# NyanCAD/CedarSim.jl

Measured on AMD Instinct MI355X. Metric: newton_iters_per_sec, higher is better.
Workload: dtype f64

## Files before the change

cedarsim.jl_amd/csrc/ch_engine.hip:

```cpp
#include <hip/hip_runtime.h>
#include <hip/hip_ext.h>

#include <algorithm>
#include <atomic>
#include <chrono>
#include <cmath>
#include <cstdio>
#include <cstring>
#include <map>
#include <memory>
#include <new>
#include <stdexcept>
#include <string>
#include <array>
#include <vector>

#include "../../include/cedarhip.h"
#include "ch_analysis.hpp"
#include "ch_bsim4.hpp"
#include "ch_dc_start.hpp"
#include "ch_device_mem.hpp"
#include "ch_env.hpp"
#include "ch_gather_plan.hpp"
#include "ch_kernels.hpp"
// ... 22 lines not shown
  const double* dev_values = nullptr; int64_t dev_n = 0;
  ch_stats stats;
  int status = CH_OK;
  int n_obs = 0, S = 1;
  std::vector<double> sens; int n_par = 0;
};

struct PersistConsts; struct PersistIo; struct PersistLaunch; struct PersistRun; struct PersistStep;
struct RowStore;
struct TranSens;
struct ch_circuit;

struct Structure {
  DevBuf<int> d_comp_class, d_comp_uofs, d_comp_dofs, d_gl_ptr, d_dkind, d_dterm, d_dsrc, d_dhdev, d_obs_unk, d_unk_obs;
  DevBuf<unsigned long long> d_stamps; DevBuf<ClassMeta> d_classes; DevBuf<unsigned char> d_dmask;
  DevBuf<int> d_dvac, d_va_mod, d_va_pofs, d_va_cofs;
  int n_va_inst = 0; size_t vac_total = 0; std::vector<ClassMeta> h_cms;
  std::vector<int> obs_primary;
  std::vector<int> needed_src;
  std::vector<int> dev_src;
  int n_dev_src() const { return std::max<int>(1, (int)dev_src.size()); }
  int block_threads = 64, lu_variant = 16;
  bool wide_split = false; int wide_l = 0, wide_other = 0;
  size_t lds_doubles_fixed = 0, lds_extra_bytes = 0, lds_plan_bytes = 0;
 private: friend struct ch_circuit;
  void class_blobs(const Description& D, std::vector<int>& blob) {
    h_cms.clear();
    int max_slots = 0;
    for (size_t ci = 0; ci < D.A.classes.size(); ++ci) {
      const CompClass& c = D.A.classes[ci];
      ClassMeta m; std::memset(&m, 0, sizeof(m));
      m.nc = c.nc; m.ndev = c.ndev; m.nonlinear = c.nonlinear ? 1 : 0;
      m.n_mat_src = (int)c.mat_src.size(); m.n_vec_src = (int)c.vec_src.size();
      while (blob.size() & 3) blob.push_back(0);
      m.blob_ofs = (int)blob.size();
      blob.insert(blob.end(), c.mat_ptr.begin(), c.mat_ptr.end());
      blob.insert(blob.end(), c.vec_ptr.begin(), c.vec_ptr.end());
      int rep = -1;
      for (int k = 0; k < D.A.n_comp; ++k) if (D.A.comp_class[k] == (int)ci) { rep = k; break; }
      int ns = 0;
      {
        std::vector<int> lanes;
        bool big = false;
        for (int d = 0; d < c.ndev; ++d) {
          const EDev& e = D.A.edev[D.A.comp_dofs[rep] + d];
          if (e.kind != K_VA) continue;
          if (va_gen::MODULES[D.dev[e.hdev].ipar[0]].n_params >= 64) big = true;
// ... 15 lines not shown
      std::vector<uint16_t> h16(c.mat_src); h16.insert(h16.end(), c.vec_src.begin(), c.vec_src.end());
      if (h16.size() & 1) h16.push_back(0);
      for (size_t i = 0; i < h16.size(); i += 2) blob.push_back((int)((uint32_t)h16[i] | ((uint32_t)h16[i + 1] << 16)));
      if (((int)blob.size() - m.blob_ofs) & 1) blob.push_back(0);
      m.wl_ofs = (int)blob.size() - m.blob_ofs;
      if (c.nc <= 64 && !c.vec_ptr.empty()) {
        std::vector<std::array<int, 3>> items;
        for (int i = 0; i < c.nc; ++i) {
          const int start = c.vec_ptr[i], cnt = c.vec_ptr[i + 1] - start;
          items.push_back({cnt, m.n_mat_src + start, (int)(0x8000u | (uint32_t)i)});
        }
        for (int e = 0; e < c.nc * c.nc; ++e) {
          const int start = c.mat_ptr[e], cnt = c.mat_ptr[e + 1] - start;
          if (cnt == 0 && e / c.nc != e % c.nc) continue;
          items.push_back({cnt, start, e});
        }
        std::stable_sort(items.begin(), items.end(), [](const std::array<int, 3>& x, const std::array<int, 3>& y) { return x[0] > y[0]; });
        for (const auto& it : items) { blob.push_back(it[1]); blob.push_back((int)(((uint32_t)it[0] << 16) | (uint32_t)it[2])); ++m.n_work; }
      }
      while ((blob.size() - m.blob_ofs) & 3) blob.push_back(0);
      m.blob_ints = (int)blob.size() - m.blob_ofs;
      if (m.n_work > 0) {
        GatherPlan gp;
        if (gp.build(c.nc, c.mat_ptr, c.vec_ptr, h16, m.n_mat_src)) {
          m.spare0 = (int)gp.words.size(); m.spare1 = gp.T;
          blob.insert(blob.end(), gp.words.begin(), gp.words.end());
        }
      }
      if (env_on(Env::DEBUG_BLOB)) std::fprintf(stderr, "[blob] class %zu: nc %d ndev %d slots %d mat_src %d vec_src %d work %d blob_ints %d trips %d\n", ci, m.nc, m.ndev, m.nslots, m.n_mat_src, m.n_vec_src, m.n_work, m.blob_ints, m.spare1);
      max_slots = std::max(max_slots, m.nslots);
      h_cms.push_back(m);
    }
    block_threads = std::min(256, std::max(64, ((max_slots + 63) / 64) * 64));
    lu_variant = D.A.max_nc <= 8 ? 8 : (D.A.max_nc <= 12 ? 12 : (D.A.max_nc <= 16 ? 16 : (D.A.max_nc <= 32 ? 32 : 0)));
    if (D.A.wide) lu_variant = D.A.max_nc <= 16 ? 16 : 0;
  }
  void source_lists(const Description& D, std::vector<int>& dkind, std::vector<int>& dterm, std::vector<int>& dhdev, std::vector<int>& dsrc) {
    dsrc.clear();
    dev_src.clear();
    { std::vector<int> slot_of(D.src.size(), -1);
      for (const EDev& e : D.A.edev) {
        dkind.push_back(e.kind); for (int k = 0; k < NTERM; ++k) dterm.push_back(e.term[k]); dhdev.push_back(e.hdev);
        int si = e.kind == K_VA ? D.dev[e.hdev].ipar[1] : 0;
        if (e.src >= 0) { if (slot_of[e.src] < 0) { slot_of[e.src] = (int)dev_src.size(); dev_src.push_back(e.src); } si = slot_of[e.src]; }
        dsrc.push_back(si);
      }
      std::vector<char> need(D.src.size(), 0);
// ... 11 lines not shown
      const int mod = D.dev[e.hdev].ipar[0];
      dvac[i] = (int)vac_total; vmod.push_back(mod); vpofs.push_back(D.dev[e.hdev].ipar[1]); vcofs.push_back((int)vac_total);
      vac_total += (size_t)va_gen::N_CACHE[mod];
    }
    n_va_inst = (int)vmod.size();
    if (vmod.empty()) { vmod.push_back(0); vpofs.push_back(0); vcofs.push_back(0); }
  }
  void masks_and_observables(const Description& D, std::vector<unsigned char>& dm, std::vector<int>& obs_unk, std::vector<int>& unk_obs) {
    dm.assign(D.A.n_unk, 0);
    for (int u = 0; u < D.A.n_unk; ++u) dm[u] = (D.A.diff_mask[u] ? 1 : 0) | (D.A.unk_mna[u] >= D.n_nodes ? 2 : 0) | (D.A.replica[u] ? 4 : 0);
    obs_unk.clear(); unk_obs.assign(D.A.n_unk, -1);
    obs_primary.clear();
    for (size_t o = 0; o < D.obs_kind.size(); ++o) {
      int u = -1;
      if (D.obs_kind[o] == 0) u = D.A.node_unknown[D.obs_index[o]];
      else { int b = D.dev[D.obs_index[o]].branch; u = b >= 0 ? D.A.branch_unknown[b] : -1; }
      obs_unk.push_back(u);
      int prim = (int)o;
      if (u >= 0) { if (unk_obs[u] < 0) unk_obs[u] = (int)o; else prim = unk_obs[u]; }
      obs_primary.push_back(prim);
    }
  }
  void size_lds(const Description& D) {
    lds_doubles_fixed = 0; lds_extra_bytes = 0; lds_plan_bytes = 0;
    for (size_t ci = 0; ci < D.A.classes.size(); ++ci) {
      const CompClass& c = D.A.classes[ci];
      lds_doubles_fixed = std::max(lds_doubles_fixed, (size_t)c.ndev * D.A.stride() + (size_t)c.nc * (c.nc + 1) + (size_t)c.nc * c.nc + 12 * (size_t)c.nc);
      lds_extra_bytes = std::max(lds_extra_bytes, ((size_t)h_cms[ci].blob_ints + 64) * 4 + 16);
      lds_plan_bytes = std::max(lds_plan_bytes, (size_t)h_cms[ci].spare0 * 4);
    }
  }
};
struct SampleTables : ParamTables {
  int S = 1; bool dirty = true;
  std::vector<std::vector<double>> slot_val;
  long vac_stride_ = 0;
  DevBuf<double> d_dpar, d_dmult, d_gmin, d_temp, d_mosp, d_vapar, d_vacache;
  DevBuf<int> d_dcls, d_moscls_inst, d_mc_ofs, d_mc_n, d_mc_list, d_dcls_local;
  DevBuf<BlockMeta> d_bmeta;
};
struct SourceTables { const std::vector<double>* dc; const std::vector<double>* par; };
struct NewtonState {
  DevBuf<double> d_X, d_Q, d_rate, d_kv;
  DevBuf<unsigned char> d_perm, d_active;
  DevBuf<BlockOut> d_out; PinnedBuf<BlockOut> h_out;
  PinnedBuf<Summary> h_sum; PinnedBuf<double> h_stage;
  DevEvent ev0, ev1; bool host_reduce = true; size_t lds_bytes = 0;
  int path = 1;
  NewtonArgs base;
  mutable std::vector<double> all_src; std::vector<double> sv_buf, kv_buf;
};
struct SpGrids { int gn, gd, ga, nbr; bool many; };
// ... 742 lines not shown
```

cedarsim.jl_amd/csrc/ch_engine_persist.hpp:

```cpp
#pragma once

constexpr size_t P_MAX_ENTRIES = 64, P_MAX_PWL = 2048;
inline bool ch_circuit::persist_eligible(std::string& why, bool own_steps) {
  auto no = [&](const char* m) { why = m; return false; };
  if (nwt.path != 1) return no("the circuit takes the sparse path");
  if (desc.A.n_comp < 1) return no("the circuit has no unknowns");
  if (!(stru.lu_variant == 8 || stru.lu_variant == 12 || stru.lu_variant == 16)) return no("a Jacobian block has more than 16 unknowns");
  if (desc.A.wide) {
    if (desc.A.classes.size() != 1) return no("compiled Verilog-A devices in blocks of several classes");
    if (desc.A.nb > 0) return no("compiled Verilog-A devices in a bordered form");
    if (stru.wide_split ? (stru.wide_l + stru.wide_other > 32) : (stru.h_cms[0].nslots > 64)) return no("a block's compiled devices need more evaluation lanes than a wave pair offers");
    if (own_steps && tab.S == 1 && desc.A.n_comp > 1) return no("per-block steps of one circuit with compiled Verilog-A devices");
  } else if (stru.block_threads != 64) return no("a block needs more than one wavefront of device slots");
  if (tab.max_mc > 8) return no("more than 8 MOSFET classes in a block");
  if (tab.Ssrc != 1) return no("per-sample source parameters");
  const bool wg_consts = own_steps && tab.S == 1 && desc.A.n_comp > 1;
  if (!wg_consts && (stru.needed_src.size() > (size_t)P_MAXSRC || desc.A.known.size() + (size_t)stru.n_dev_src() > P_MAX_ENTRIES)) return no("more than 64 sources / known-node and source values per attempt");
  if (!(tab.S == 1 || desc.A.n_comp == 1)) return no("several blocks per sample in a multi-sample batch");
  if (desc.A.nb > 0 && (tab.S != 1 || desc.A.border_dev.size() > 8)) return no("bordered form: one sample and at most 8 devices on the border alone");
  for (const ClassMeta& m : stru.h_cms) if ((!desc.A.wide && m.nslots > 64) || m.nc > stru.lu_variant || m.n_work <= 0 || m.spare1 <= 0) return no("a block class does not fit the one-wave register path");
  if (ps.n_cu == 0) { hipDeviceProp_t prop; if (hipGetDeviceProperties(&prop, ctx->device) != hipSuccess) return no("hipGetDeviceProperties failed"); ps.n_cu = prop.multiProcessorCount; }
  const long nblk = (long)desc.A.n_comp * tab.S;
  const int bpw = persist_bpw(nblk);
  if (nblk > (long)bpw * ps.n_cu && !own_steps) return no("more blocks than resident wavefronts (4 per CU)");
  if (!own_steps && (nblk + bpw - 1) / bpw > 256) return no("more than 256 workgroups in a grid-wide reduction");
  size_t npwl = 0; for (int i : stru.needed_src) npwl += desc.src[i].ts.size();
  if (!wg_consts && npwl > P_MAX_PWL) return no("piecewise-linear tables above 2048 points");
  return true;
}
inline int ch_circuit::persist_bpw(long nblk) const {
  if (ps.n_cu > 0 && desc.A.wide && stru.wide_split && nblk <= 2L * ps.n_cu) return 2;
  return PW;
}
inline bool ch_circuit::persist_own_steps(const ch_tran_opts& o) const {
  return ((desc.A.n_comp == 1 && tab.S > 1) || (tab.S == 1 && desc.A.n_comp > 1 && desc.A.nb == 0 && !desc.A.wide)) && o.n_saveat > 0 && o.step_control != CH_STEPS_SHARED && !env_on(Env::LOCKSTEP);
}
inline size_t ch_circuit::persist_wave_doubles(bool wg_consts) const {
  const size_t n_ent = wg_consts ? (size_t)P_MAXSRC : desc.A.known.size() + stru.n_dev_src();
  return stru.lds_doubles_fixed + 16 * (size_t)desc.A.max_nc + 10 + 48 + P_MAXSRC + n_ent + (size_t)tab.max_mc * (B4L_STRIDE + B4D_STRIDE) + (stru.lds_extra_bytes + stru.lds_plan_bytes + 7) / 8 + 2;
}
inline bool ch_circuit::persist_blob(const std::vector<int>& kn, const std::vector<int>& ds, std::vector<int>& bi, std::vector<double>& bd, std::vector<int>& need) const {
  const int nsrc = (int)desc.src.size();
  std::vector<char> nd(std::max(1, nsrc), 0);
  for (int k : kn) for (auto& tm : desc.A.known[k].terms) nd[tm.first] = 1;
  for (int j : ds) if (j < (int)stru.dev_src.size()) nd[stru.dev_src[j]] = 1;
  need.clear();
  for (int i = 0; i < nsrc; ++i) if (nd[i]) need.push_back(i);
  std::vector<int> pos(std::max(1, nsrc), -1);
  for (size_t i = 0; i < need.size(); ++i) pos[need[i]] = (int)i;
  std::vector<double> pt, py;
  bi = {(int)need.size(), (int)(kn.size() + ds.size()), 0, (int)kn.size()};
  for (int i : need) { bi.push_back(desc.src[i].kind); bi.push_back((int)pt.size()); bi.push_back((int)desc.src[i].ts.size()); pt.insert(pt.end(), desc.src[i].ts.begin(), desc.src[i].ts.end()); py.insert(py.end(), desc.src[i].ys.begin(), desc.src[i].ys.end()); }
  bi[2] = (int)pt.size();
  std::vector<int> eptr(1, 0), eidx; std::vector<double> ecoef;
  for (int k : kn) { for (auto& tm : desc.A.known[k].terms) { eidx.push_back(pos[tm.first]); ecoef.push_back(tm.second); } eptr.push_back((int)eidx.size()); }
  for (int j : ds) { if (j < (int)stru.dev_src.size()) { eidx.push_back(pos[stru.dev_src[j]]); ecoef.push_back(1.0); } eptr.push_back((int)eidx.size()); }
  bi.insert(bi.end(), eptr.begin(), eptr.end()); bi.insert(bi.end(), eidx.begin(), eidx.end());
  bd.clear();
  for (int i : need) for (int k = 0; k < CH_SRC_NPAR; ++k) bd.push_back(tab.src_par[(size_t)i * CH_SRC_NPAR + k]);
  bd.insert(bd.end(), ecoef.begin(), ecoef.end()); bd.insert(bd.end(), pt.begin(), pt.end()); bd.insert(bd.end(), py.begin(), py.end());
  for (size_t q = 4; q < bi.size(); ++q) if (bi[q] < 0) return false;
  return need.size() <= (size_t)P_MAXSRC && kn.size() + ds.size() <= P_MAX_ENTRIES && pt.size() <= P_MAX_PWL;
// ... 226 lines not shown
  pa.indep = L.own_steps ? 1 : 0;
  ps.mode = desc.A.nb > 0 ? CH_MODE_BORDERED : (L.own_steps ? CH_MODE_OWN_STEPS : CH_MODE_LOCKSTEP);
  if (dcm) {
    if (desc.A.nb == 0 || L.wg_consts) { set_err("internal: operating point on the device stepper is for the bordered form"); return CH_ERR_INTERNAL; }
    std::vector<double> sv, kv, ent;
    eval_sources(0.0, dcm->tran_mode ? 2 : 0, sv, kv);
    ent.assign(kv.begin(), kv.begin() + nk); ent.insert(ent.end(), sv.begin(), sv.begin() + nds);
    HIPCHK(ps.d_pdcent.upload(ent, ctx->stream));
    pa.dc_mode = 1; pa.dc_maxit = std::max(1, dcm->maxiters); pa.dc_abstol = dcm->abstol; pa.dc_entries = ps.d_pdcent.p;
    pa.dv_max = (!desc.A.mos_hdev.empty() || desc.A.wide) ? dcm->dv_max : 0.0;
  }
  pa.nb = desc.A.nb; pa.n_glob = desc.A.n_glob; pa.n_bdev = (int)desc.A.border_dev.size();
  for (int q = 0; q < pa.n_bdev; ++q) {
    const Analysis::BorderDev& bd = desc.A.border_dev[q];
    pa.bd_kind[q] = bd.kind; pa.bd_ta[q] = bd.ta; pa.bd_tb[q] = bd.tb;
    const double par0 = tab.dpar[(size_t)bd.hdev * tab.Spar], mult0 = tab.dmult[(size_t)bd.hdev * tab.Spar];
    pa.bd_val[q] = bd.kind == K_R ? mult0 / par0 : mult0 * par0;
  }
  pa.pair_dbg = (int)env_long(Env::PAIR_DBG, 0);
  return CH_OK;
}
inline PersistStep ch_circuit::persist_pick_kernel(PersistLaunch& L) {
  const int mode = desc.A.wide ? (L.own_steps ? PM_OWN : PM_LOCKSTEP) : desc.A.nb > 0 ? PM_BORDER : (L.own_steps ? PM_OWN : PM_LOCKSTEP);
  L.fn = persist_kernel(desc.A.wide, mode, (desc.A.wide || desc.A.nb > 0 || stru.lu_variant > 12) ? 16 : 12, L.pair);
  if (!L.fn) { set_err("internal: no device-stepper kernel for this form"); return CH_ERR_INTERNAL; }
  if (ps.attr_fn != L.fn) {
    hipFuncAttributes fa;
    HIPCHK(hipFuncGetAttributes(&fa, L.fn));
    if (fa.sharedSizeBytes <= 160 * 1024) HIPCHK(hipFuncSetAttribute(L.fn, hipFuncAttributeMaxDynamicSharedMemorySize, (int)((160 * 1024 - (int)fa.sharedSizeBytes) & ~255)));
    ps.attr_static_lds = fa.sharedSizeBytes; ps.attr_fn = L.fn;
  }
  if (L.lds + ps.attr_static_lds > 160 * 1024) { set_err("device-resident stepper: LDS footprint"); return PersistStep::declined(); }
  return CH_OK;
}
inline PersistStep ch_circuit::persist_prepare(const TranPlan& p, const ch_dc_opts* dcm, PersistLaunch& L) {
  const ch_tran_opts& o = *p.o;
  g_arena = &arena;
  LapTimer lt(host_profile);
  L.nblk = desc.A.n_comp * tab.S; L.bpw = persist_bpw(L.nblk); L.n_wg = (L.nblk + L.bpw - 1) / L.bpw;
  L.own_steps = persist_own_steps(o);
  L.wg_consts = L.own_steps && tab.S == 1 && desc.A.n_comp > 1;
  PersistConsts pc;
  if (!persist_consts(L.wg_consts, L.n_wg, L.bpw, p, pc)) return PersistStep::declined();
  L.wave_d = persist_wave_doubles(L.wg_consts);
  L.lds = (pc.max_cd + (pc.max_ci + 1) / 2 + PW * P_NREC + P_NREC + 4 + P_SCR + PW * L.wave_d) * sizeof(double);
  L.va_arena = persist_va_arena(L.bpw, L.lds);
  L.pair = desc.A.wide ? stru.wide_split : (desc.A.classes.size() == 1 && stru.h_cms[0].nslots <= 32 && !env_on(Env::PERSIST_NOPAIR));
// ... 172 lines not shown
```

cedarsim.jl_amd/csrc/ch_gather_plan.hpp:

```cpp
#pragma once
#include <algorithm>
#include <array>
#include <cstdint>
#include <vector>

namespace chip {

constexpr int GP_HEAD_INTS = 64;
constexpr unsigned GP_N_MASK = 7u, GP_END = 8u, GP_VEC = 16u;
constexpr int GP_A_SHIFT = 6, GP_C_SHIFT = 19;
constexpr unsigned GP_OFS_MASK = 0x1fffu;

struct GatherPlan {
  struct Item { int first, cnt, code; };
  int T = 0;
  int n_items = 0, total_trips = 0, max_item_trips = 0;
  int R = 0;
  std::vector<int> words;
  std::vector<int> item_lane, item_trip;
  std::vector<Item> items;

  static int trips_of(int cnt) { return cnt <= 0 ? 1 : (cnt + 3) / 4; }
  static int lower_bound_T(int total_trips, int max_item_trips) { return std::max((total_trips + 63) / 64, max_item_trips); }

  static std::vector<Item> class_items(int nc, const std::vector<int>& mat_ptr, const std::vector<int>& vec_ptr, int n_mat_src) {
    std::vector<Item> it;
    for (int i = 0; i < nc; ++i) it.push_back({n_mat_src + vec_ptr[i], vec_ptr[i + 1] - vec_ptr[i], (int)(0x8000u | (uint32_t)i)});
    for (int e = 0; e < nc * nc; ++e) {
      const int cnt = mat_ptr[e + 1] - mat_ptr[e];
      if (cnt == 0 && e / nc != e % nc) continue;
      it.push_back({mat_ptr[e], cnt, e});
    }
    std::stable_sort(it.begin(), it.end(), [](const Item& x, const Item& y) { return x.cnt > y.cnt; });
    return it;
  }

  bool build(int nc, const std::vector<int>& mat_ptr, const std::vector<int>& vec_ptr, const std::vector<uint16_t>& src16, int n_mat_src) {
    T = 0; R = 0; n_items = 0; total_trips = 0; max_item_trips = 0; words.clear(); item_lane.clear(); item_trip.clear(); items.clear();
    if (nc < 1 || nc > 64 || (int)vec_ptr.size() != nc + 1 || (int)mat_ptr.size() != nc * nc + 1) return false;
    items = class_items(nc, mat_ptr, vec_ptr, n_mat_src);
    n_items = (int)items.size();
    for (const Item& it : items) { total_trips += trips_of(it.cnt); max_item_trips = std::max(max_item_trips, trips_of(it.cnt)); }
    std::vector<int> order(n_items);
    for (int i = 0; i < n_items; ++i) order[i] = i;
    std::stable_sort(order.begin(), order.end(), [&](int x, int y) { return trips_of(items[x].cnt) > trips_of(items[y].cnt); });
    std::array<int, 64> load;
    for (int t = lower_bound_T(total_trips, max_item_trips);; ++t) {
      load.fill(0);
      item_lane.assign(n_items, -1); item_trip.assign(n_items, 0);
      bool ok = true;
      for (int i : order) {
        const int s = trips_of(items[i].cnt);
        int l = 0;
        while (l < 64 && load[l] + s > t) ++l;
        if (l == 64) { ok = false; break; }
        item_lane[i] = l; item_trip[i] = load[l]; load[l] += s;
      }
      if (ok) { T = t; break; }
    }
    std::array<int, 64> base;
    { int next = 1; for (int l = 0; l < 64; ++l) { base[l] = load[l] > 0 ? next : 0; next += load[l]; } R = (next + 3) & ~3; }
    const int lda = nc + 1;
    words.assign((size_t)GP_HEAD_INTS + 3 * (size_t)R, 0);
    int* src = words.data() + GP_HEAD_INTS; int* ctl = src + 2 * (size_t)R;
    for (int l = 0; l < 64; ++l) words[l] = (int)((uint32_t)base[l] | ((uint32_t)load[l] << 16));
    for (int i = 0; i < n_items; ++i) {
      const Item& it = items[i];
      const int l = item_lane[i], s = trips_of(it.cnt);
      const bool vec = (it.code & 0x8000) != 0;
      const int e = it.code & 0x7fff;
      const unsigned oa = vec ? (unsigned)(e * lda + nc) : (unsigned)((e / nc) * lda + e % nc);
      const unsigned oc = vec ? (unsigned)(nc * nc + 3 * nc + e) : (unsigned)e;
      for (int q = 0; q < s; ++q) {
        const int rec = base[l] + item_trip[i] + q;
        const int left = it.cnt - 4 * q, n = left < 0 ? 0 : (left > 4 ? 4 : left);
        uint16_t o[4] = {0, 0, 0, 0};
        for (int k = 0; k < n; ++k) o[k] = src16[(size_t)it.first + 4 * q + k];
        src[2 * rec] = (int)((uint32_t)o[0] | ((uint32_t)o[1] << 16));
        src[2 * rec + 1] = (int)((uint32_t)o[2] | ((uint32_t)o[3] << 16));
        unsigned c = (unsigned)n | (vec ? GP_VEC : 0u);
        if (q == s - 1) c |= GP_END | (oa << GP_A_SHIFT) | (oc << GP_C_SHIFT);
        ctl[rec] = (int)c;
      }
    }
    if (R > 0xffff || T > 0xffff) return false;
    return true;
  }
};

}
```

cedarsim.jl_amd/csrc/ch_kernels.hpp:

```cpp
#pragma once
#include <hip/hip_runtime.h>

#include "ch_analysis.hpp"
#include "ch_bsim4.hpp"
#include "ch_param_tables.hpp"
#include "_generated/va_models.hpp"

namespace chip {


struct BlockOut {
  int status;
  int iters;
  int ndiff;
  int pad;
  double e2k, e2km1, e2kp1;
  double fnorm;
};

struct Summary {
  int n_fail, max_iters, n_singular, pad;
  long long sum_iters;
  long long sum_block_iters;
  double errk, errkm1, errkp1;
// ... 352 lines not shown
#pragma unroll
  for (int k = NC - 1; k >= 0; --k) {
    if (k < nc) {
      const double xk = bcast(rhs * ipiv, piv[k]);
      if (lane == k) out = xk;
      if (mystep >= 0 && mystep < k) rhs = fma(-r[k], xk, rhs);
    }
  }
  sol = out;
  if (myrow_out) {
    int mr = lane;
#pragma unroll
    for (int k = 0; k < NC; ++k) if (k < nc && lane == k) mr = piv[k];
    *myrow_out = mr;
  }
  return true;
}

template <int K> __device__ __forceinline__ double row_bcast(double v) {
  static_assert(K >= 0 && K < 16, "row_newbcast lane");
  const double b = __builtin_amdgcn_update_dpp(v, v, 0x150 + K, 0xF, 0xF, true);
  return b;
}
template <int NC, int J> struct RowDot {
  static __device__ __forceinline__ double run(const double (&c)[NC], double x, int nc, double q) {
    if constexpr (J < NC) {
      if (J < nc) { const double xj = row_bcast<J>(x); q = fma(c[J], xj, q); }
      return RowDot<NC, J + 1>::run(c, x, nc, q);
    } else return q;
  }
};

template <int NC, int K>
struct LuStaticStep {
  static __device__ __forceinline__ void fwd(double (&r)[NC + 1], int nc, int lane, int& lkey, double& ipiv) {
    if constexpr (K < NC) {
      if (K < nc) {
        const double ipk = frcp(row_bcast<K>(r[K]));
        double pj[NC + 1];
#pragma unroll
        for (int j = K + 1; j <= NC; ++j) pj[j] = row_bcast<K>(r[j]);
        if (lane == K) ipiv = ipk;
        if (lane > K) {
          const double l = r[K] * ipk;
          lkey = max(lkey, __double2hiint(l) & 0x7fffffff);
#pragma unroll
          for (int j = K + 1; j <= NC; ++j) r[j] = fma(-l, pj[j], r[j]);
        }
      }
      LuStaticStep<NC, K + 1>::fwd(r, nc, lane, lkey, ipiv);
    }
  }
  static __device__ __forceinline__ void bwd(const double (&r)[NC + 1], int nc, int lane, double& rhs, double ipiv) {
    if constexpr (K < NC) {
      constexpr int Q = NC - 1 - K;
      if (Q < nc && Q > 0) {
        const double xk = row_bcast<Q>(rhs * ipiv);
        if (lane < Q) rhs = fma(-r[Q], xk, rhs);
      }
      LuStaticStep<NC, K + 1>::bwd(r, nc, lane, rhs, ipiv);
    }
  }
};
template <int NC>
__device__ __forceinline__ bool lu_solve_static(double (&r)[NC + 1], int nc, int lane_in, double& sol) {
  static_assert(NC <= 16, "row_newbcast spans one 16-lane row");
  int lane = lane_in;
  asm volatile("" : "+v"(lane));
  int lkey = 0; double ipiv = 0.0;
  LuStaticStep<NC, 0>::fwd(r, nc, lane, lkey, ipiv);
  if (__ballot(lane < nc && lkey > 0x40200000)) return false;
  double rhs = r[NC];
  LuStaticStep<NC, 0>::bwd(r, nc, lane, rhs, ipiv);
  sol = rhs * ipiv;
  return true;
}
struct LuFull { double sol; int myrow; int ok; };
template <int NC>
__device__ __attribute__((noinline, cold)) LuFull lu_solve_full(const double* A, int lda, int nc, int lane, int myrow) {
  double r[NC + 1];
#pragma unroll
  for (int j = 0; j <= NC; ++j) r[j] = (lane < nc && j <= nc) ? A[lane * lda + j] : 0.0;
  LuFull o; o.sol = 0.0; o.myrow = myrow;
  o.ok = lu_solve_regs<NC>(r, nc, lane, o.sol, &o.myrow) ? 1 : 0;
  return o;
}
template <int NC>
__device__ __forceinline__ bool lu_solve_block(const double* A, int lda, int nc, int lane_in, int& myrow, double& sol) {
  if constexpr (NC <= 16) {
    int lane = lane_in;
    asm volatile("" : "+v"(lane));
    const int lim = lane < nc ? nc : 0;
    const double* row = A + (lim > 0 ? myrow : 0) * lda;
    double r[NC + 1];
#pragma unroll
    for (int j = 0; j < NC; ++j) { const double v = row[j]; r[j] = j < lim ? v : 0.0; }
    { const double v = row[nc]; r[NC] = lim > 0 ? v : 0.0; }
    if (lu_solve_static<NC>(r, nc, lane_in, sol)) return true;
    const LuFull f = lu_solve_full<NC>(A, lda, nc, lane_in, myrow);
    myrow = f.myrow; sol = f.sol;
    return f.ok != 0;
  } else {
    double r[NC + 1];
#pragma unroll
    for (int j = 0; j <= NC; ++j) r[j] = (lane_in < nc && j <= nc) ? A[lane_in * lda + j] : 0.0;
    return lu_solve_regs<NC>(r, nc, lane_in, sol, &myrow);
  }
}

template <int NC>
__device__ __forceinline__ bool lu_bbd_factor(double (&r)[NC + 1], int no, int nc, int lane, int (&piv)[NC], int& mystep, double& ipiv) {
// ... 663 lines not shown
```

cedarsim.jl_amd/csrc/ch_persist.hpp:

```cpp
#pragma once
#include <hip/hip_runtime.h>

#include "ch_gather_plan.hpp"
#include "ch_kernels.hpp"

#ifdef CH_STAMPS
#define P_STAMP(slot) do { const unsigned long long now_ = __builtin_readcyclecounter(); pacc_[slot] += now_ - plast_; plast_ = now_; } while (0)
#else
#define P_STAMP(slot) do { } while (0)
#endif

namespace chip {

constexpr int PW = 4;
constexpr int P_MAXSRC = 64;
constexpr int P_NREC = 8;
constexpr int P_SCR = 64;
enum { PX_RUNNING = 0, PX_DONE = 1, PX_ROWS_FULL = 2, PX_ABORT = 3 };

struct TranCtl {
  double t, h;
  double tslot[8];
  int k, nhist, steps_at_order, reset_rate;
  int ibp, isave, status, exit_reason;
// ... 293 lines not shown
    const int* e = wgc + 6 * wg;
    const int* gci = p.ci + e[0]; const double* gcd = p.cd + e[1]; const int n_ci = e[2], n_cd = e[3];
    bps_own = p.bps + e[4]; nbp_own = e[5];
    for (int i = tid; i < n_cd; i += PW * 64) cdl[i] = gcd[i];
    for (int i = tid; i < n_ci; i += PW * 64) cil[i] = gci[i];
  } else {
    for (int i = tid; i < p.n_cd; i += PW * 64) cdl[i] = p.cd[i];
    for (int i = tid; i < p.n_ci; i += PW * 64) cil[i] = p.ci[i];
  }
#define P_BPS ((own && wgc) ? bps_own : p.bps)
#define P_NBP ((own && wgc) ? nbp_own : p.nbp)
  if (tid == 0) s_abort = 0;
  if (tid < 8) pfl[tid] = 0;
  const KLds kpool = kpool_fill(s_kpool, tid);
  __syncthreads();
  const PConst C{cil, cdl};

  const int blk = wg * p.bpw + wave;
  const bool live = wave < p.bpw && blk < p.nblk;
  const int bq = live ? blk : 0;
  const int c = bq / a.S, s = bq - c * a.S;
  const BlockMeta bm = a.bmeta[c];
  const ClassMeta cm = bm.cm;
  const int nc = cm.nc, ndev = cm.ndev, uofs = bm.uofs, dofs = bm.dofs, lda = nc + 1;
  double* st = W;
  double* A = st + (size_t)ndev * SL::STRIDE;
  double* Cm = A + (size_t)nc * lda;
  double* xl = Cm + (size_t)nc * nc;
  double* xp = xl + nc; double* Fv = xp + nc; double* Qv = Fv + nc; double* hq = Qv + nc;
  double* wv = hq + nc; double* qn = wv + nc; double* pm = qn + nc; double* pp = pm + nc; double* x0l = pp + nc;
  int* dml = (int*)(x0l + nc);
  double* Xh = x0l + 2 * nc; double* Qh = Xh + 8 * nc;
  double* tsl = Qh + 8 * nc; double* coef = tsl + 8;
  long long* stl = (long long*)(coef + 40);
  double* kvl = coef + 48; double* svl = kvl + (wgc ? C.ci[3] : a.nk);
  double* pl = wgc ? kvl + P_MAXSRC : svl + a.nsrc;
  double* dl = pl + (size_t)a.max_mc * B4L_STRIDE;
  int* mptr = (int*)(dl + (size_t)a.max_mc * B4D_STRIDE);
  int* slots = mptr + (nc * nc + 1) + (nc + 1);
  const int* gplan = mptr + cm.blob_ints;
  const int g_recs = (cm.spare0 - GP_HEAD_INTS) / 3;
  const uint2* gsrc = (const uint2*)(gplan + GP_HEAD_INTS);
  const unsigned* gctl = (const unsigned*)(gplan + GP_HEAD_INTS + 2 * g_recs);
  const int g_trips = __builtin_amdgcn_readfirstlane(cm.spare1);
  const long sofs = (long)s * a.n_unk + uofs;
  const bool mine = live && lane < nc;
  const int nc_s = __builtin_amdgcn_readfirstlane(nc);
  const int role = wave & 1, pairq = wave >> 1, half = lane >> 5;
  int* pf = pfl + pairq * 4;
  const int blk_h = wg * p.bpw + (wave & ~1) + half;
  const bool live_h = PAIR && (wave & ~1) + half < p.bpw && blk_h < p.nblk;
// ... 17 lines not shown
      __builtin_amdgcn_s_sleep(0);
    }
    lds_fence();
  };

  if (live) {
    const int* bsrc = a.blob + cm.blob_ofs;
    for (int i = lane; i < cm.blob_ints + cm.spare0; i += 64) mptr[i] = bsrc[i];
    const long scol = a.Smos > 1 ? s : 0;
    const int total = bm.mc_n * B4I_COUNT;
    for (int e = lane; e < total; e += 64) {
      const int j = e / B4I_COUNT, i = e - j * B4I_COUNT;
      int cl = bm.mc[0];
#pragma unroll
      for (int q = 1; q < 8; ++q) cl = (j == q) ? bm.mc[q] : cl;
      pl[j * B4L_STRIDE + i] = a.mosp[((long)cl * a.Smos + scol) * (long)B4I_COUNT + i];
    }
    lds_fence();
    if (lane < bm.mc_n) {
      const B4Col Pj{pl + (size_t)lane * B4L_STRIDE};
#pragma unroll
      for (int e = 0; e < B4D_COUNT; ++e) dl[(size_t)lane * B4D_STRIDE + e] = b4_derive(Pj, e);
    }
    for (int i = lane; i < nc * lda + nc * nc; i += 64) A[i] = 0.0;
    if (mine) {
      dml[lane] = a.dmask[uofs + lane] | ((a.unk_obs[uofs + lane] + 1) << 8);
#pragma unroll
      for (int j = 0; j < 7; ++j) {
        const bool have = j < p.ctl->nhist;
        Xh[((8 - j) & 7) * nc + lane] = have ? a.X[(long)j * a.slot_stride + sofs + lane] : 0.0;
        Qh[((8 - j) & 7) * nc + lane] = have ? a.Qh[(long)j * a.slot_stride + sofs + lane] : 0.0;
      }
      Xh[1 * nc + lane] = 0.0; Qh[1 * nc + lane] = 0.0;
    }
  }
  if (lane < 8) tsl[(8 - lane) & 7] = p.ctl->tslot[lane];
  {
    const double nd = row_sum<16>((mine && (dml[lane] & 1)) ? 1.0 : 0.0);
    if (lane == 0) coef[35] = nd;
  }
  double t, h; int k, nhist, steps_at_order, ibp, isave, status = CH_OK, exit_reason = PX_RUNNING;
  bool reset_rate;
  int nsaved, step;
  enum { ST_ACC = 0, ST_REJ, ST_FAIL, ST_ITERS, ST_BITERS, ST_ATT };
  int head = 0;
  {
// ... 257 lines not shown
              if (vec) {
                const double F = G + hqe;
                Cm[oc - nc_s] = F;
                A[oa] = -F;
              } else A[oa] = G;
              Cm[oc] = s2;
              s1 = 0.0; s2 = 0.0;
            }
          }
        }
        lds_fence();
        P_STAMP(5);
        constexpr int NCR = NC;
        double r[NCR + 1], cr[NCR];
        if constexpr (MODE == PM_BORDER) {
#pragma unroll
          for (int j = 0; j <= NCR; ++j) r[j] = (mine && j <= nc) ? A[lane * lda + j] : 0.0;
        }
        int lr = lane;
        asm volatile("" : "+v"(lr));
        const int rlim = ((bbd ? live : true) && lr < nc) ? nc : 0;
        const int rrow = rlim > 0 ? lr : 0;
        {
          const double* crow = Cm + rrow * nc_s;
#pragma unroll
          for (int j = 0; j < NCR; ++j) { const double v = crow[j]; cr[j] = j < rlim ? v : 0.0; }
        }
        const double Fr = Fv[rrow], Qr = Qv[rrow], xr_ = xl[rrow], wr = wv[rrow];
        const double Fi = rlim > 0 ? Fr : 0.0, Qi = rlim > 0 ? Qr : 0.0, xi = rlim > 0 ? xr_ : 0.0, wi = rlim > 0 ? wr : 0.0;
        const double fnorm = bcast(row_max<NCR>(fabs(Fi)), 0);
        if (bbd) {
          bool lfail = live && (!(fnorm == fnorm) || fnorm > 1e300 || dc_bad);
          const double fown = bcast(row_max<NCR>((mine && lane < no) ? fabs(Fi) : 0.0), 0);
          int piv[NCR]; int mystep; double ipiv;
          if (!lu_bbd_factor<NCR>(r, no, nc, lane, piv, mystep, ipiv)) lfail = live;
          double srec[P_NREC];
          {
            double c0 = 0.0, c1 = 0.0, cr_ = 0.0;
#pragma unroll
            for (int j = 0; j <= NCR; ++j) { if (j == no) c0 = r[j]; if (j == no + 1 && j < nc) c1 = r[j]; if (j == nc) cr_ = r[j]; }
            const bool use = live && !lfail;
            srec[0] = use ? bcast(c0, no) : 0.0; srec[1] = use ? bcast(c1, no) : 0.0; srec[2] = use ? bcast(cr_, no) : 0.0;
            const int l1 = p.nb > 1 ? no + 1 : no;
            srec[3] = (use && p.nb > 1) ? bcast(c0, l1) : 0.0; srec[4] = (use && p.nb > 1) ? bcast(c1, l1) : 0.0; srec[5] = (use && p.nb > 1) ? bcast(cr_, l1) : 0.0;
            srec[6] = (lfail ? 1.0 : 0.0) + (pair_broken ? 1048576.0 : 0.0);
            srec[7] = (dcm && live && !(fown < p.dc_abstol)) ? 1.0 : 0.0;
          }
          ++gen;
          const long long cbA = wall_clock64();
// ... 98 lines not shown
          const long long cbB = wall_clock64();
          okr = p_grid_reduce<true>(p, gen, brec, part, summ, &s_abort, wave, lane, wg);
          bA = summ[0]; bB = summ[1]; bC = summ[2]; bN = summ[3];
          const double e2g = summ[4]; const bool gbad = summ[5] != 0.0;
          if (!okr || summ[7] != 0.0) abort_all = true;
          __syncthreads();
          cyc_bar += wall_clock64() - cbB;
          if (abort_all) break;
          if (gbad) { nstat = 2; break; }
          const double dn = sqrt(e2g / (double)p.n_glob);
          if (it == 0) { if (dn <= a.newton_tol || (rp < 0.9 && 2.0 * fmax(rp, 0.02) * dn <= a.newton_tol)) { nstat = 0; stop_all = true; } }
          else { rate_new = dn_prev > 0.0 ? dn / dn_prev : 0.0; if (dn <= a.newton_tol) { nstat = 0; stop_all = true; } }
          dn_prev = dn;
          if (it + 1 >= a.maxit) stop_all = true;
          lds_fence();
          continue;
        }
        bool stop = false;
        if (!(fnorm == fnorm) || fnorm > 1e300) { nstat = 2; stop = true; }
        else if (it == a.maxit) { stop = true; }
        else {
          double dx = 0.0;
          P_STAMP(6);
          const bool ok = lu_solve_block<NCR>(A, lda, nc, lane, myrow, dx);
          P_STAMP(7);
          if (!ok) { nstat = 2; stop = true; }
          else {
            const double xn = xi + dx;
            if (mine) xl[lane] = xn;
            const bool bad = mine && (!(xn == xn) || fabs(xn) > 1e300);
            const double tq = dx * wi;
            const double e2 = bcast(row_sum<NCR>(mine ? tq * tq : 0.0), 0);
            const double q = RowDot<NCR, 0>::run(cr, dx, nc, Qi);
            if (mine) qn[lane] = q;
            ++iters;
            if (__ballot(bad)) { nstat = 2; stop = true; }
            else {
              const double dn = sqrt(e2 / nc);
              if (it == 0) { if (dn <= a.newton_tol || (rp < 0.9 && 2.0 * fmax(rp, 0.02) * dn <= a.newton_tol)) { nstat = 0; stop = true; } }
              else { rate_new = dn_prev > 0.0 ? dn / dn_prev : 0.0; if (dn <= a.newton_tol) { nstat = 0; stop = true; } }
              dn_prev = dn;
            }
          }
        }
        lds_fence();
        P_STAMP(8);
        if (stop) { if (PAIR) done_own = true; else break; }
      }
    }
    if (dcm) {
      if (abort_all) { exit_reason = PX_ABORT; status = CH_ERR_DEVICE; break; }
      if (mine) Xh[head * nc + lane] = xl[lane];
      if (lane == 0) { stl[ST_ITERS] += iters; stl[ST_BITERS] += (long long)iters * p.nblk; }
      lds_fence();
      status = nstat == 0 ? CH_OK : (nstat == 2 ? CH_ERR_SINGULAR : CH_ERR_MAXITERS);
      exit_reason = PX_DONE;
// ... 178 lines not shown
```

Measured before the change: 61170.

## Pad per-block Jacobian to compile-time width for branch-free static LU

Lays out the block Jacobian and capacitance matrices in LDS with a fixed compile-time stride (NC+1, NC) instead of the runtime nc, and fills the padded rows with identity so the LU, back-substitution and row-dot loops can drop their runtime `K < nc` guards. The gather plan is rebuilt with the padded strides, and the kernel selection now comes from a shared helper. This removes per-step predicates and dynamic indexing in the Newton solve. The cost is extra LDS per wave, which may lower occupancy, plus extra work on padded rows when nc is below NC.

```diff
diff --git a/cedarsim.jl_amd/csrc/ch_engine.hip b/cedarsim.jl_amd/csrc/ch_engine.hip
--- a/cedarsim.jl_amd/csrc/ch_engine.hip
+++ b/cedarsim.jl_amd/csrc/ch_engine.hip
@@ -68,7 +68,7 @@
   int n_dev_src() const { return std::max<int>(1, (int)dev_src.size()); }
   int block_threads = 64, lu_variant = 16;
   bool wide_split = false; int wide_l = 0, wide_other = 0;
-  size_t lds_doubles_fixed = 0, lds_extra_bytes = 0, lds_plan_bytes = 0;
+  size_t lds_doubles_fixed = 0, lds_extra_bytes = 0, lds_plan_bytes = 0, lds_pad_doubles = 0;
  private: friend struct ch_circuit;
   void class_blobs(const Description& D, std::vector<int>& blob) {
     h_cms.clear();
@@ -130,7 +130,7 @@
       m.blob_ints = (int)blob.size() - m.blob_ofs;
       if (m.n_work > 0) {
         GatherPlan gp;
-        if (gp.build(c.nc, c.mat_ptr, c.vec_ptr, h16, m.n_mat_src)) {
+        if (gp.build(c.nc, c.mat_ptr, c.vec_ptr, h16, m.n_mat_src, GatherStrides::of(D.A.wide, D.A.nb, D.A.max_nc, c.nc))) {
           m.spare0 = (int)gp.words.size(); m.spare1 = gp.T;
           blob.insert(blob.end(), gp.words.begin(), gp.words.end());
         }
@@ -188,12 +188,13 @@
     }
   }
   void size_lds(const Description& D) {
-    lds_doubles_fixed = 0; lds_extra_bytes = 0; lds_plan_bytes = 0;
+    lds_doubles_fixed = 0; lds_extra_bytes = 0; lds_plan_bytes = 0; lds_pad_doubles = 0;
     for (size_t ci = 0; ci < D.A.classes.size(); ++ci) {
       const CompClass& c = D.A.classes[ci];
       lds_doubles_fixed = std::max(lds_doubles_fixed, (size_t)c.ndev * D.A.stride() + (size_t)c.nc * (c.nc + 1) + (size_t)c.nc * c.nc + 12 * (size_t)c.nc);
       lds_extra_bytes = std::max(lds_extra_bytes, ((size_t)h_cms[ci].blob_ints + 64) * 4 + 16);
       lds_plan_bytes = std::max(lds_plan_bytes, (size_t)h_cms[ci].spare0 * 4);
+      lds_pad_doubles = std::max(lds_pad_doubles, (size_t)GatherStrides::of(D.A.wide, D.A.nb, D.A.max_nc, c.nc).extra_doubles(c.nc));
     }
   }
 };
diff --git a/cedarsim.jl_amd/csrc/ch_engine_persist.hpp b/cedarsim.jl_amd/csrc/ch_engine_persist.hpp
--- a/cedarsim.jl_amd/csrc/ch_engine_persist.hpp
+++ b/cedarsim.jl_amd/csrc/ch_engine_persist.hpp
@@ -37,7 +37,7 @@
 }
 inline size_t ch_circuit::persist_wave_doubles(bool wg_consts) const {
   const size_t n_ent = wg_consts ? (size_t)P_MAXSRC : desc.A.known.size() + stru.n_dev_src();
-  return stru.lds_doubles_fixed + 16 * (size_t)desc.A.max_nc + 10 + 48 + P_MAXSRC + n_ent + (size_t)tab.max_mc * (B4L_STRIDE + B4D_STRIDE) + (stru.lds_extra_bytes + stru.lds_plan_bytes + 7) / 8 + 2;
+  return stru.lds_doubles_fixed + stru.lds_pad_doubles + 16 * (size_t)desc.A.max_nc + 10 + 48 + P_MAXSRC + n_ent + (size_t)tab.max_mc * (B4L_STRIDE + B4D_STRIDE) + (stru.lds_extra_bytes + stru.lds_plan_bytes + 7) / 8 + 2;
 }
 inline bool ch_circuit::persist_blob(const std::vector<int>& kn, const std::vector<int>& ds, std::vector<int>& bi, std::vector<double>& bd, std::vector<int>& need) const {
   const int nsrc = (int)desc.src.size();
@@ -310,7 +310,7 @@
 }
 inline PersistStep ch_circuit::persist_pick_kernel(PersistLaunch& L) {
   const int mode = desc.A.wide ? (L.own_steps ? PM_OWN : PM_LOCKSTEP) : desc.A.nb > 0 ? PM_BORDER : (L.own_steps ? PM_OWN : PM_LOCKSTEP);
-  L.fn = persist_kernel(desc.A.wide, mode, (desc.A.wide || desc.A.nb > 0 || stru.lu_variant > 12) ? 16 : 12, L.pair);
+  L.fn = persist_kernel(desc.A.wide, mode, persist_lu_nc(desc.A.wide, desc.A.nb, desc.A.max_nc), L.pair);
   if (!L.fn) { set_err("internal: no device-stepper kernel for this form"); return CH_ERR_INTERNAL; }
   if (ps.attr_fn != L.fn) {
     hipFuncAttributes fa;
diff --git a/cedarsim.jl_amd/csrc/ch_gather_plan.hpp b/cedarsim.jl_amd/csrc/ch_gather_plan.hpp
--- a/cedarsim.jl_amd/csrc/ch_gather_plan.hpp
+++ b/cedarsim.jl_amd/csrc/ch_gather_plan.hpp
@@ -10,6 +10,18 @@
 constexpr unsigned GP_N_MASK = 7u, GP_END = 8u, GP_VEC = 16u;
 constexpr int GP_A_SHIFT = 6, GP_C_SHIFT = 19;
 constexpr unsigned GP_OFS_MASK = 0x1fffu;
+
+inline int persist_lu_nc(bool wide, int nb, int max_nc) { return max_nc > 16 ? 0 : ((wide || nb > 0 || max_nc > 12) ? 16 : 12); }
+struct GatherStrides {
+  int lda, ldc;
+  static GatherStrides unpadded(int nc) { return {nc + 1, nc}; }
+  static GatherStrides of(bool wide, int nb, int max_nc, int nc) {
+    const int NC = persist_lu_nc(wide, nb, max_nc);
+    return (NC == 0 || nb > 0 || nc > NC) ? unpadded(nc) : GatherStrides{NC + 1, NC};
+  }
+  bool padded(int nc) const { return lda != nc + 1; }
+  int extra_doubles(int nc) const { return padded(nc) ? (lda - 1) * lda + nc * ldc - nc * (nc + 1) - nc * nc : 0; }
+};
 
 struct GatherPlan {
   struct Item { int first, cnt, code; };
@@ -36,8 +48,12 @@
   }
 
   bool build(int nc, const std::vector<int>& mat_ptr, const std::vector<int>& vec_ptr, const std::vector<uint16_t>& src16, int n_mat_src) {
+    return build(nc, mat_ptr, vec_ptr, src16, n_mat_src, GatherStrides::unpadded(nc));
+  }
+  bool build(int nc, const std::vector<int>& mat_ptr, const std::vector<int>& vec_ptr, const std::vector<uint16_t>& src16, int n_mat_src, GatherStrides gs) {
     T = 0; R = 0; n_items = 0; total_trips = 0; max_item_trips = 0; words.clear(); item_lane.clear(); item_trip.clear(); items.clear();
     if (nc < 1 || nc > 64 || (int)vec_ptr.size() != nc + 1 || (int)mat_ptr.size() != nc * nc + 1) return false;
+    if (gs.lda <= nc || gs.ldc < nc) return false;
     items = class_items(nc, mat_ptr, vec_ptr, n_mat_src);
     n_items = (int)items.size();
     for (const Item& it : items) { total_trips += trips_of(it.cnt); max_item_trips = std::max(max_item_trips, trips_of(it.cnt)); }
@@ -60,7 +76,7 @@
     }
     std::array<int, 64> base;
     { int next = 1; for (int l = 0; l < 64; ++l) { base[l] = load[l] > 0 ? next : 0; next += load[l]; } R = (next + 3) & ~3; }
-    const int lda = nc + 1;
+    const int lda = gs.lda, ldc = gs.ldc;
     words.assign((size_t)GP_HEAD_INTS + 3 * (size_t)R, 0);
     int* src = words.data() + GP_HEAD_INTS; int* ctl = src + 2 * (size_t)R;
     for (int l = 0; l < 64; ++l) words[l] = (int)((uint32_t)base[l] | ((uint32_t)load[l] << 16));
@@ -69,8 +85,8 @@
       const int l = item_lane[i], s = trips_of(it.cnt);
       const bool vec = (it.code & 0x8000) != 0;
       const int e = it.code & 0x7fff;
-      const unsigned oa = vec ? (unsigned)(e * lda + nc) : (unsigned)((e / nc) * lda + e % nc);
-      const unsigned oc = vec ? (unsigned)(nc * nc + 3 * nc + e) : (unsigned)e;
+      const unsigned oa = vec ? (unsigned)(e * lda + lda - 1) : (unsigned)((e / nc) * lda + e % nc);
+      const unsigned oc = vec ? (unsigned)(nc * ldc + 3 * nc + e) : (unsigned)((e / nc) * ldc + e % nc);
       for (int q = 0; q < s; ++q) {
         const int rec = base[l] + item_trip[i] + q;
         const int left = it.cnt - 4 * q, n = left < 0 ? 0 : (left > 4 ? 4 : left);
@@ -83,6 +99,7 @@
         ctl[rec] = (int)c;
       }
     }
+    if ((unsigned)(nc * lda) > GP_OFS_MASK || (unsigned)(nc * ldc + 4 * nc) > GP_OFS_MASK) return false;
     if (R > 0xffff || T > 0xffff) return false;
     return true;
   }
diff --git a/cedarsim.jl_amd/csrc/ch_kernels.hpp b/cedarsim.jl_amd/csrc/ch_kernels.hpp
--- a/cedarsim.jl_amd/csrc/ch_kernels.hpp
+++ b/cedarsim.jl_amd/csrc/ch_kernels.hpp
@@ -398,20 +398,20 @@
   const double b = __builtin_amdgcn_update_dpp(v, v, 0x150 + K, 0xF, 0xF, true);
   return b;
 }
-template <int NC, int J> struct RowDot {
+template <int NC, int J, bool PAD = false> struct RowDot {
   static __device__ __forceinline__ double run(const double (&c)[NC], double x, int nc, double q) {
     if constexpr (J < NC) {
-      if (J < nc) { const double xj = row_bcast<J>(x); q = fma(c[J], xj, q); }
-      return RowDot<NC, J + 1>::run(c, x, nc, q);
+      if (PAD || J < nc) { const double xj = row_bcast<J>(x); q = fma(c[J], xj, q); }
+      return RowDot<NC, J + 1, PAD>::run(c, x, nc, q);
     } else return q;
   }
 };
 
-template <int NC, int K>
+template <int NC, int K, bool PAD = false>
 struct LuStaticStep {
   static __device__ __forceinline__ void fwd(double (&r)[NC + 1], int nc, int lane, int& lkey, double& ipiv) {
     if constexpr (K < NC) {
-      if (K < nc) {
+      if (PAD || K < nc) {
         const double ipk = frcp(row_bcast<K>(r[K]));
         double pj[NC + 1];
 #pragma unroll
@@ -424,30 +424,30 @@
           for (int j = K + 1; j <= NC; ++j) r[j] = fma(-l, pj[j], r[j]);
         }
       }
-      LuStaticStep<NC, K + 1>::fwd(r, nc, lane, lkey, ipiv);
+      LuStaticStep<NC, K + 1, PAD>::fwd(r, nc, lane, lkey, ipiv);
     }
   }
   static __device__ __forceinline__ void bwd(const double (&r)[NC + 1], int nc, int lane, double& rhs, double ipiv) {
     if constexpr (K < NC) {
       constexpr int Q = NC - 1 - K;
-      if (Q < nc && Q > 0) {
+      if ((PAD || Q < nc) && Q > 0) {
         const double xk = row_bcast<Q>(rhs * ipiv);
         if (lane < Q) rhs = fma(-r[Q], xk, rhs);
       }
-      LuStaticStep<NC, K + 1>::bwd(r, nc, lane, rhs, ipiv);
+      LuStaticStep<NC, K + 1, PAD>::bwd(r, nc, lane, rhs, ipiv);
     }
   }
 };
-template <int NC>
+template <int NC, bool PAD = false>
 __device__ __forceinline__ bool lu_solve_static(double (&r)[NC + 1], int nc, int lane_in, double& sol) {
   static_assert(NC <= 16, "row_newbcast spans one 16-lane row");
   int lane = lane_in;
   asm volatile("" : "+v"(lane));
   int lkey = 0; double ipiv = 0.0;
-  LuStaticStep<NC, 0>::fwd(r, nc, lane, lkey, ipiv);
+  LuStaticStep<NC, 0, PAD>::fwd(r, nc, lane, lkey, ipiv);
   if (__ballot(lane < nc && lkey > 0x40200000)) return false;
   double rhs = r[NC];
-  LuStaticStep<NC, 0>::bwd(r, nc, lane, rhs, ipiv);
+  LuStaticStep<NC, 0, PAD>::bwd(r, nc, lane, rhs, ipiv);
   sol = rhs * ipiv;
   return true;
 }
@@ -462,7 +462,29 @@
   return o;
 }
 template <int NC>
+__device__ __attribute__((noinline, cold)) LuFull lu_solve_full_padded(const double* A, int nc, int lane, int myrow) {
+  double r[NC + 1];
+#pragma unroll
+  for (int j = 0; j <= NC; ++j) r[j] = (lane < nc && j <= nc) ? A[lane * (NC + 1) + (j == nc ? NC : j)] : 0.0;
+  LuFull o; o.sol = 0.0; o.myrow = myrow;
+  o.ok = lu_solve_regs<NC>(r, nc, lane, o.sol, &o.myrow) ? 1 : 0;
+  return o;
+}
+template <int NC, bool PAD = false>
 __device__ __forceinline__ bool lu_solve_block(const double* A, int lda, int nc, int lane_in, int& myrow, double& sol) {
+  if constexpr (PAD) {
+    static_assert(NC <= 16, "the padded solve is the register LU with a static pivot order");
+    int lane = lane_in;
+    asm volatile("" : "+v"(lane));
+    const double* row = A + (lane < NC ? myrow : 0) * (NC + 1);
+    double r[NC + 1];
+#pragma unroll
+    for (int j = 0; j <= NC; ++j) r[j] = row[j];
+    if (lu_solve_static<NC, true>(r, nc, lane_in, sol)) return true;
+    const LuFull f = lu_solve_full_padded<NC>(A, nc, lane_in, myrow);
+    myrow = f.myrow; sol = f.sol;
+    return f.ok != 0;
+  } else
   if constexpr (NC <= 16) {
     int lane = lane_in;
     asm volatile("" : "+v"(lane));
diff --git a/cedarsim.jl_amd/csrc/ch_persist.hpp b/cedarsim.jl_amd/csrc/ch_persist.hpp
--- a/cedarsim.jl_amd/csrc/ch_persist.hpp
+++ b/cedarsim.jl_amd/csrc/ch_persist.hpp
@@ -339,11 +339,14 @@
   const int c = bq / a.S, s = bq - c * a.S;
   const BlockMeta bm = a.bmeta[c];
   const ClassMeta cm = bm.cm;
-  const int nc = cm.nc, ndev = cm.ndev, uofs = bm.uofs, dofs = bm.dofs, lda = nc + 1;
+  const int nc = cm.nc, ndev = cm.ndev, uofs = bm.uofs, dofs = bm.dofs;
+  constexpr bool PAD = MODE != PM_BORDER;
+  static_assert(NC <= 16, "one 16-lane row holds the block");
+  const int lda = PAD ? NC + 1 : nc + 1, ldc = PAD ? NC : nc;
   double* st = W;
   double* A = st + (size_t)ndev * SL::STRIDE;
-  double* Cm = A + (size_t)nc * lda;
-  double* xl = Cm + (size_t)nc * nc;
+  double* Cm = A + (size_t)(PAD ? NC : nc) * lda;
+  double* xl = Cm + (size_t)nc * ldc;
   double* xp = xl + nc; double* Fv = xp + nc; double* Qv = Fv + nc; double* hq = Qv + nc;
   double* wv = hq + nc; double* qn = wv + nc; double* pm = qn + nc; double* pp = pm + nc; double* x0l = pp + nc;
   int* dml = (int*)(x0l + nc);
@@ -407,6 +410,10 @@
 #pragma unroll
       for (int e = 0; e < B4D_COUNT; ++e) dl[(size_t)lane * B4D_STRIDE + e] = b4_derive(Pj, e);
     }
+    if (PAD) {
+      for (int i = lane; i < NC * (NC + 1); i += 64) { const int row = i / (NC + 1); A[i] = (row >= nc && i - row * (NC + 1) == row) ? 1.0 : 0.0; }
+      for (int i = lane; i < nc * NC; i += 64) Cm[i] = (i % NC >= nc) ? -0.0 : 0.0;
+    } else
     for (int i = lane; i < nc * lda + nc * nc; i += 64) A[i] = 0.0;
     if (mine) {
       dml[lane] = a.dmask[uofs + lane] | ((a.unk_obs[uofs + lane] + 1) << 8);
@@ -710,9 +717,9 @@
         const int rlim = ((bbd ? live : true) && lr < nc) ? nc : 0;
         const int rrow = rlim > 0 ? lr : 0;
         {
-          const double* crow = Cm + rrow * nc_s;
-#pragma unroll
-          for (int j = 0; j < NCR; ++j) { const double v = crow[j]; cr[j] = j < rlim ? v : 0.0; }
+          const double* crow = Cm + rrow * (PAD ? NC : nc_s);
+#pragma unroll
+          for (int j = 0; j < NCR; ++j) { const double v = crow[j]; cr[j] = (PAD || j < rlim) ? v : 0.0; }
         }
         const double Fr = Fv[rrow], Qr = Qv[rrow], xr_ = xl[rrow], wr = wv[rrow];
         const double Fi = rlim > 0 ? Fr : 0.0, Qi = rlim > 0 ? Qr : 0.0, xi = rlim > 0 ? xr_ : 0.0, wi = rlim > 0 ? wr : 0.0;
@@ -857,7 +864,7 @@
         else {
           double dx = 0.0;
           P_STAMP(6);
-          const bool ok = lu_solve_block<NCR>(A, lda, nc, lane, myrow, dx);
+          const bool ok = lu_solve_block<NCR, PAD>(A, lda, nc, lane, myrow, dx);
           P_STAMP(7);
           if (!ok) { nstat = 2; stop = true; }
           else {
@@ -866,7 +873,7 @@
             const bool bad = mine && (!(xn == xn) || fabs(xn) > 1e300);
             const double tq = dx * wi;
             const double e2 = bcast(row_sum<NCR>(mine ? tq * tq : 0.0), 0);
-            const double q = RowDot<NCR, 0>::run(cr, dx, nc, Qi);
+            const double q = RowDot<NCR, 0, PAD>::run(cr, dx, nc, Qi);
             if (mine) qn[lane] = q;
             ++iters;
             if (__ballot(bad)) { nstat = 2; stop = true; }
```

Result: faster. 63690 (median of 6 runs) (+4.1%).
